# 1dayac/spades_for_blackbird

Hardware: AMD Instinct MI355X
Metric: distinct k-mers/sec (k=21, 150 bp synthetic reads, count only) (higher is better)
Workload: dtype u64

## Files before the change

spades_for_blackbird_amd/build.py:

```python
import os
import subprocess
import sys
from concurrent.futures import ThreadPoolExecutor

HERE = os.path.dirname(os.path.abspath(__file__))
CSRC = os.path.join(HERE, "csrc")
LIB = os.path.join(HERE, "libbbk.so")
SOURCES = ["pool.hip", "context.hip", "scan.hip", "sort.hip", "unique.hip", "msd.hip", "superk.hip", "reads.hip", "count.hip", "extindex.hip", "tipclip.hip", "atclip.hip", "readfilter.hip", "unitigs.hip", "unitigs_write.hip", "edgeprof.hip", "kmerprof.hip", "hamclust.hip", "kmerstat.hip", "subclust.hip", "expand.hip", "readcorrect.hip", "hreads.hip", "readprint.hip", "group.hip", "fastqparse.hip", "kmerfilter.hip"]
HEADERS = ["bbk_internal.h", "block_scan.h", "kmer_ops.h", "extwalk.h", "msd.h", "msd_part.h", "msd_bucket.h", "msd_narrow_a.h", "msd_stage_b.h", "msd_bucket_tail.h", "accum.h", "arena.h", "select.h", "unitigs.h", "hammer.h", "hammer_files.h", "readcorrect_host.hpp", os.path.join("..", "host", "hammer_reads.hpp"), "gfa_graph.h", os.path.join("..", "..", "include", "bbk.h")]
ARCH = "gfx950"
FLAGS = ["-O3", "-std=c++17", "-fPIC", "--offload-arch=" + ARCH, "-fopenmp", "-Wall", "-Wno-unused-function"]


def _hipcc():
    for c in (os.environ.get("HIPCC"), "/opt/rocm/bin/hipcc", "hipcc"):
        if c and (os.path.isabs(c) and os.path.exists(c) or not os.path.isabs(c)):
            return c
    raise RuntimeError("hipcc not found")


def _stale(target, deps):
    if not os.path.exists(target):
        return True
    t = os.path.getmtime(target)
# ... 119 lines not shown
```

spades_for_blackbird_amd/csrc/msd.hip:

```cpp
#include <hip/hip_runtime.h>

#include <algorithm>
#include <chrono>
#include <cmath>
#include <cstdio>
#include <cstdlib>
#include <cstring>
#include <optional>
#include <type_traits>
#include <utility>
#include <vector>

#include "bbk_internal.h"
#include "kmer_ops.h"
#include "msd.h"
#include "msd.h"

#include "msd_part.h"
#include "msd_bucket.h"
#include "msd_narrow_a.h"
#include "msd_stage_b.h"

namespace bbk {

// ... 518 lines not shown
                         v.slots.as<uint32_t>(), v.off.as<uint64_t>(), v.seg.as<uint16_t>(), vdesc.template as<uint2>(),
                         v.stride, v.hb, Mv, L1, cur1.as<uint32_t>(), bufA.as<Key<1>>());
            }
            if (v.n_extra) {
                TileMap Me = M1;
                Me.n = 2 * v.n_extra;
                const uint32_t nte = (uint32_t)((Me.n + kPartTileK - 1) / kPartTileK);
                R.template scatter_keys<true>(false, "k_part_l1", rec_bytes(v.n_extra) + rec_bytes(Me.n), nte,
                                              v.extra.as<Key<W>>(), nullptr, Me, L1, cur1.as<uint32_t>(),
                                              bufA.as<Key<W>>(), nullptr);
            }
        }

        void level1_late_tag(BucketView &v) {
            constexpr uint32_t kpt = (uint32_t)kLtThreads * kLt1Items / 2;
            const size_t lds = lt_smem(kLt1Items, (size_t)kViewSpan * (4 + 2));
            ctx->add_stat("stat_late_tag", (double)N);
            const auto [vdesc, nt] = view_tiles(v, kpt);
            if (nt)
                R.launch(k_part_view_lt<false>, "k_part_view", (double)v.D * 4 + 2.0 * (double)v.D * 4, nt, kLtThreads, lds,
                         v.slots.as<uint32_t>(), v.off.as<uint64_t>(), v.seg.as<uint16_t>(), vdesc.template as<uint2>(),
                         v.stride, v.hb, (const uint64_t *)nullptr, v.D, (int)R.expand_k, L1, cur1.as<uint32_t>(),
                         bufA.as<uint32_t>());
            if (v.n_extra) {
                const uint32_t nte = (uint32_t)((v.n_extra + kpt - 1) / kpt);
                R.launch(k_part_view_lt<true>, "k_part_l1", (double)v.n_extra * 8 + 2.0 * (double)v.n_extra * 4, nte,
                         kLtThreads, lds, (const uint32_t *)nullptr, (const uint64_t *)nullptr, (const uint16_t *)nullptr,
                         (const uint2 *)nullptr, 0u, 0, v.extra.as<uint64_t>(), v.n_extra, (int)R.expand_k, L1,
                         cur1.as<uint32_t>(), bufA.as<uint32_t>());
            }
        }
// ... 1042 lines not shown
```

spades_for_blackbird_amd/csrc/msd_narrow_a.h:

```cpp
#pragma once

namespace bbk {

constexpr int kNwBins1 = 1024;
__device__ inline uint32_t nw_mix(uint32_t lo) {
    uint32_t t = lo * 0x9E3779B1u;
    t ^= t >> 15;
    t *= 0x85EBCA6Bu;
    t ^= t >> 13;
    return t;
}
__device__ inline uint32_t nw_slot(uint32_t t) { return (t * 0x27D4EB2Fu) >> 19; }
__device__ inline uint32_t nw_bin1(uint32_t hi, uint32_t t, int hb) { return (t >> 22) ^ (hi << (10 - hb)); }
__device__ inline uint32_t nw_p2(uint32_t t) { return t << 10; }
__device__ inline uint32_t nw_bin2(uint32_t t, uint32_t nb) {
#ifdef BBK_AB_NW_BIN2_MULHI
    return __umulhi(nw_p2(t), nb);
#else
    return __umul24(t & 0x3FFFFFu, nb) >> 22;
#endif
}
__device__ inline uint64_t nw_key(uint32_t bin1, uint32_t lo, int hb) {
    const uint32_t hi = (bin1 ^ (nw_mix(lo) >> 22)) >> (10 - hb);
    return ((uint64_t)hi << 32) | lo;
// ... 127 lines not shown
        for (int i = 0; i < CH; ++i) lo[r * CH + i] = l8[i];
#pragma unroll
        for (int i = 0; i < 3; ++i) bins[r * 3 + i] = b3[i];
        masks[r * 2] = m2[0];
        masks[r * 2 + 1] = m2[1];
        cnts |= cnt << (4 * r);
    }
}

template <bool HAS_VAL>
__global__ __launch_bounds__(kNwThreads) __attribute__((amdgpu_waves_per_eu(BBK_NW_WAVES, BBK_NW_WAVES))) void k_part_reads_narrow(ReadSrc S, PartLevel L, uint32_t ntiles,
                                                                 const RdTile *__restrict__ tiles_arg,
                                                                 uint32_t *__restrict__ cursor,
                                                                 uint32_t *__restrict__ out, uint32_t *__restrict__ vout) {
    constexpr int NT = kNwThreads, CH = 8, MAXB = kNwBins1, ITEMS = CH * NwCfg<HAS_VAL>::ROUNDS;
    constexpr int MW = NwCfg<HAS_VAL>::TILE / 64;
    extern __shared__ __attribute__((aligned(16))) unsigned char smem[];
    uint32_t *lhist = reinterpret_cast<uint32_t *>(smem);
    uint2 *tab = reinterpret_cast<uint2 *>(smem);
    uint32_t *lstart = lhist + 2 * MAXB;
    uint32_t *scan_tmp = lstart + MAXB;
    unsigned long long *mark = reinterpret_cast<unsigned long long *>(scan_tmp + 64);
    uint16_t *mbase = reinterpret_cast<uint16_t *>(mark + MW);
    uint16_t *nz = mbase + MW;
    unsigned char *U = reinterpret_cast<unsigned char *>(nz + MAXB);
    int32_t *s_rel = reinterpret_cast<int32_t *>(U);
    int32_t *s_wrel = s_rel + (kRdSlots + 2);
    uint32_t *s_len = reinterpret_cast<uint32_t *>(s_wrel + (kRdSlots + 2));
    uint64_t *s_words = reinterpret_cast<uint64_t *>(s_len + (kRdSlots + 2));
    uint32_t *stage = reinterpret_cast<uint32_t *>(U);
    uint8_t *vstage = reinterpret_cast<uint8_t *>(stage + NwCfg<HAS_VAL>::TILE);

    uint32_t tid = threadIdx.x;
    const uint32_t k_ = (uint32_t)S.k;
    const int hb = L.narrow_hb;
    uint32_t xcc = 0;
    if (L.xcd_shift) {
        asm volatile("s_getreg_b32 %0, hwreg(HW_REG_XCC_ID)" : "=s"(xcc));
        xcc &= (1u << L.xcd_shift) - 1u;
    }
#ifdef BBK_PHASE_PROF
    unsigned long long t_prev = clock64();
#else
    const unsigned long long t_prev = 0;
    (void)t_prev;
#endif
// ... 16 lines not shown
    };

#ifdef BBK_NW_TILES_VIA_STRUCT
    const RdTile *tiles = S.tiles;
    (void)tiles_arg;
#else
    const RdTile *__restrict__ tiles = tiles_arg;
#endif
    uint32_t tile = blockIdx.x;
    if (tile >= ntiles) return;
    RdTile T = tiles[tile];
    Pre Q{0, 0, 0, 0, 0};
    prefetch(T, Q);
    for (;;) {
        asm volatile("" : "+v"(tid));
        const int lane = tid & 63, wave = tid >> 6;
        const uint32_t tile_next = tile + gridDim.x;
        const bool more = tile_next < ntiles;
        RdTile Tn = T;
        if (more) Tn = tiles[tile_next];

        const uint64_t c0 = (uint64_t)tile * NwCfg<HAS_VAL>::CHUNKS;
        const uint64_t left = S.n_chunks - c0;
        const uint32_t nch = left < (uint64_t)NwCfg<HAS_VAL>::CHUNKS ? (uint32_t)left : (uint32_t)NwCfg<HAS_VAL>::CHUNKS;
        const uint32_t r0 = T.r0, nr = T.nr;
        const uint64_t wbase = T.wbase;
        const bool fast = staged_ok(T);
        lhist[tid] = 0;
        if (tid < 2 * MW) reinterpret_cast<uint32_t *>(mark)[tid] = 0u;
        if (fast) {
            if (tid <= nr) s_rel[tid] = (int32_t)(int64_t)(Q.coff - c0);
            if (tid < nr) {
                s_wrel[tid] = (int32_t)(int64_t)(Q.woff - wbase);
                s_len[tid] = Q.len;
            }
            if (tid < T.wspan) s_words[tid] = Q.w0;
            if (tid + NT < T.wspan) s_words[tid + NT] = Q.w1;
        }
        __syncthreads();
        BBK_PH(5, 0, t_prev);

        uint32_t lo[ITEMS], bins[3 * NwCfg<HAS_VAL>::ROUNDS], masks[2 * NwCfg<HAS_VAL>::ROUNDS], cnts;
        if (fast) nw_extract<true, HAS_VAL>(S, L, k_, tid, nch, c0, r0, nr, s_rel, s_wrel, s_len, s_words, lhist, lo, bins, masks, cnts);
        else nw_extract<false, HAS_VAL>(S, L, k_, tid, nch, c0, r0, nr, s_rel, s_wrel, s_len, s_words, lhist, lo, bins, masks, cnts);
        __syncthreads();
        BBK_PH(5, 1, t_prev);

        const uint32_t c = lhist[tid];
        uint32_t incl = c;
        incl = wave_scan_incl(incl);
        const unsigned long long nzb = __ballot(c != 0);
        if (lane == 63) scan_tmp[wave] = incl | ((uint32_t)__popcll(nzb) << 16);
        __syncthreads();
        uint32_t before, total;
        wave_totals<NT / 64>(scan_tmp, lane, wave, before, total);
        const uint32_t staged = total & 0xFFFFu;
        const uint32_t ex = (before & 0xFFFFu) + incl - c;
        const uint32_t myr = (before >> 16) + (uint32_t)__popcll(nzb & ((1ull << lane) - 1ull));
        lstart[tid] = ex;
        uint32_t greserve = 0;
        if (c) {
            greserve = atomicAdd(&cursor[(tid << L.xcd_shift) + xcc], c);
            nz[myr] = (uint16_t)tid;
            atomicOr(&mark[ex >> 6], 1ull << (ex & 63u));
        }
        __syncthreads();
        BBK_PH(5, 2, t_prev);
#pragma unroll
        for (int i = 0; i < ITEMS; ++i) {
            const int r = i / CH, j = i % CH;
            if ((uint32_t)j < ((cnts >> (4 * r)) & 15u)) {
                const uint32_t bin = (bins[r * 3 + j / 3] >> (10 * (j % 3))) & 1023u;
                const uint32_t pos = atomicAdd(&lstart[bin], 1u);
                stage[pos] = lo[i];
                if (HAS_VAL) vstage[pos] = (uint8_t)(masks[r * 2 + (j >> 2)] >> (8 * (j & 3)));
            }
        }
        asm volatile("" : "+v"(greserve));
        if (c) {
            const uint64_t slot_end = L.xcd_shift ? (uint64_t)tid * L.slot_stride + (uint64_t)(xcc + 1u) * L.sub_cap
                                                  : (uint64_t)tid * L.slot_stride + L.slot_cap;
            const int64_t room = (int64_t)slot_end - (int64_t)greserve;
            tab[myr] = make_uint2(greserve - ex,
                                  (uint32_t)(int32_t)(room < -(int64_t)0x7FFF0000 ? -(int64_t)0x7FFF0000 : room) + ex);
        }
        if (wave == 0) {
            constexpr int WPL = (MW + 63) / 64;
            uint32_t pw[WPL], tot = 0;
#pragma unroll
            for (int j = 0; j < WPL; ++j) {
                const int idx = lane * WPL + j;
                pw[j] = tot;
                tot += idx < MW ? (uint32_t)__popcll(mark[idx]) : 0u;
            }
            uint32_t inc2 = tot;
            inc2 = wave_scan_incl(inc2);
            const uint32_t lb = inc2 - tot;
#pragma unroll
            for (int j = 0; j < WPL; ++j) {
                const int idx = lane * WPL + j;
                if (idx < MW) mbase[idx] = (uint16_t)(lb + pw[j]);
            }
        }
        __syncthreads();
        BBK_PH(5, 3, t_prev);
        if (more) prefetch(Tn, Q);
        else Q = Pre{0, 0, 0, 0, 0};
        const unsigned long long upto = (2ull << lane) - 1ull;
        const unsigned long long *wmark = mark + wave;
        const uint16_t *wmbase = mbase + wave;
        uint32_t full = 0;
#pragma unroll
        for (int i = 0; i < ITEMS; ++i) {
            const uint32_t pos = (uint32_t)i * NT + tid;
            if (pos < staged) {
                const uint32_t r = (uint32_t)wmbase[i * (NT / 64)] + (uint32_t)__popcll(wmark[i * (NT / 64)] & upto) - 1u;
                unsigned long long e = reinterpret_cast<const unsigned long long *>(tab)[r];
                const uint32_t rec = stage[pos];
                asm volatile("" : "+v"(e));
                if ((int32_t)pos >= (int32_t)(uint32_t)(e >> 32)) {
                    full |= 1u << i;
                } else {
                    const uint32_t g = (uint32_t)e + pos;
                    out[g] = rec;
                    if (HAS_VAL) vout[g] = vstage[pos];
                }
            }
        }
        if (full) {
#pragma unroll 1
            for (int i = 0; i < ITEMS; ++i) {
                if ((full >> i) & 1u) {
                    const uint32_t pos = (uint32_t)i * NT + tid;
                    const uint32_t r = (uint32_t)wmbase[i * (NT / 64)] + (uint32_t)__popcll(wmark[i * (NT / 64)] & upto) - 1u;
                    const uint32_t sp = atomicAdd(L.spill_count, 1u);
                    if (sp < L.spill_cap) {
                        reinterpret_cast<uint64_t *>(L.spill_keys)[sp] = nw_key(nz[r], stage[pos], hb);
                        if (HAS_VAL) L.spill_vals[sp] = vstage[pos];
                    }
                }
            }
        }
        BBK_PH(5, 4, t_prev);
#ifdef BBK_PHASE_PROF
        if (threadIdx.x == 0) atomicAdd(&g_phase[5][7], 1ull);
#endif
        if (!more) break;
        __syncthreads();
        tile = tile_next;
        T = Tn;
    }
}

static size_t part_reads_narrow_smem(bool has_val) {
    const size_t tables = sizeof(uint32_t) * 3 * (kRdSlots + 2) + sizeof(uint64_t) * (kRdWords + 1 + 2);
    const size_t tile = has_val ? NwCfg<true>::TILE : NwCfg<false>::TILE;
    const size_t stage = tile * (has_val ? 5 : 4);
    const size_t fixed = sizeof(uint32_t) * (3 * kNwBins1 + 64) + (tile / 64) * (8 + 2) + (size_t)kNwBins1 * 2;
    return fixed + std::max(tables, stage);
}

constexpr int kNw2Threads = 1024;
template <bool HAS_VAL>
struct Nw2Cfg {
    static constexpr int ITEMS = HAS_VAL ? 8 : 12;
    static constexpr int TILE = kNw2Threads * ITEMS;
};

template <bool HAS_VAL>
__global__ __launch_bounds__(kNw2Threads) void k_part_narrow2(const uint32_t *__restrict__ in, const uint32_t *__restrict__ vin,
                                                             const uint4 *__restrict__ desc, PartLevel L,
                                                             uint32_t *__restrict__ cursor, uint32_t *__restrict__ out,
                                                             uint32_t *__restrict__ vout) {
    constexpr int NT = kNw2Threads, ITEMS = Nw2Cfg<HAS_VAL>::ITEMS, MAXB = kMaxBins;
// ... 429 lines not shown
```

spades_for_blackbird_amd/csrc/msd_stage_b.h:

```cpp
#pragma once

#include "msd_bucket_tail.h"

namespace bbk {

__global__ void k_bucket_base(const uint32_t *__restrict__ seg_nb2, const uint32_t *__restrict__ seg_bin, uint32_t nseg,
                              uint32_t nbuckets, int b1, int w0bits, uint64_t *__restrict__ base) {
    const uint32_t g = blockIdx.x * blockDim.x + threadIdx.x;
    if (g >= nbuckets) return;
    const uint32_t lo = last_le(seg_bin, nseg, g);
    const uint64_t P = 1ull << (32 - b1), nb = seg_nb2[lo], j = g - seg_bin[lo];
    const uint64_t p = lo * P + (j * P + nb - 1) / nb;
    base[g] = w0bits > 32 ? p << (w0bits - 32) : 0ull;
}

template <int NT, int ITEMS>
__global__ __launch_bounds__(NT) __attribute__((amdgpu_waves_per_eu(8, 8))) void k_bucket_dist_nb(const uint32_t *__restrict__ buf, const uint64_t *__restrict__ base,
                                                       BucketArgs A) {
    constexpr int CAP = NT * ITEMS;
    constexpr int NWAVES = NT / 64;
    constexpr int DB = DistBins<1, 0>::N;
    constexpr int BPT = DB / NT;
    extern __shared__ __attribute__((aligned(16))) unsigned char smem[];
    uint32_t *bins = reinterpret_cast<uint32_t *>(smem);
// ... 328 lines not shown
            keep = !kmer_less_nucl<1>(kmer_rc<1>(x, k), x);
        }
        const uint64_t bal = __ballot(keep);
        uint32_t base = 0;
        if (lane == 0 && bal) base = atomicAdd(count, (uint32_t)__popcll(bal));
        base = __shfl(base, 0);
        const uint64_t at = (uint64_t)base + __popcll(bal & ((1ull << lane) - 1ull));
        if (keep && at < cap) out[at] = x.w[0];
    }
}

constexpr int kLtThreads = 1024;
constexpr int kLt1Items = 14;
constexpr int kLt2Items = 12;

struct LtLds {
    uint32_t *lhist;
    uint2 *tab;
    uint32_t *lstart, *scan_tmp;
    unsigned long long *mark;
    uint16_t *mbase, *nz;
    uint32_t *stage;
};
template <int ITEMS>
__device__ __forceinline__ LtLds lt_lds(unsigned char *smem) {
    constexpr int MW = kLtThreads * ITEMS / 64;
    LtLds S;
    S.lhist = reinterpret_cast<uint32_t *>(smem);
    S.tab = reinterpret_cast<uint2 *>(smem);
    S.lstart = S.lhist + 2 * kMaxBins;
    S.scan_tmp = S.lstart + kMaxBins;
    S.mark = reinterpret_cast<unsigned long long *>(S.scan_tmp + 64);
    S.mbase = reinterpret_cast<uint16_t *>(S.mark + MW);
    S.nz = S.mbase + MW;
    S.stage = reinterpret_cast<uint32_t *>(S.nz + kMaxBins);
    return S;
}
static size_t lt_smem(int items, size_t more) {
    const size_t tile = (size_t)kLtThreads * items;
    return sizeof(uint32_t) * (3 * kMaxBins + 64) + (tile / 64) * (8 + 2) + (size_t)kMaxBins * 2 + tile * 4 + more;
}

__device__ inline uint64_t lt_tagged(uint32_t seg, uint32_t lo, int lobits, int k) {
    Key<1> x;
    x.w[0] = ((uint64_t)seg << lobits) | lo;
    return x.w[0] | (__umul64hi(xxh3_64<1>(x), 16ull) << (2 * k));
}

template <int ITEMS, class KeyOf>
__device__ __forceinline__ void lt_tail(const LtLds &S, const uint32_t (&lo)[ITEMS], const uint32_t (&bins)[ITEMS / 2],
                                        uint32_t nb, uint32_t *__restrict__ cur, uint64_t slot_end, uint32_t rec_or,
                                        const PartLevel &L, uint32_t *__restrict__ out, KeyOf key_of) {
    constexpr int NT = kLtThreads, MW = NT * ITEMS / 64;
    static_assert(ITEMS % 2 == 0 && ITEMS <= 32 && NT * ITEMS < 65536, "packed bins, one bit per item, 16-bit positions");
    const uint32_t tid = threadIdx.x;
    const int lane = tid & 63, wave = tid >> 6;
    const uint32_t c = tid < nb ? S.lhist[tid] : 0u;
    uint32_t incl = c;
    incl = wave_scan_incl(incl);
    const unsigned long long nzb = __ballot(c != 0);
    if (lane == 63) S.scan_tmp[wave] = incl | ((uint32_t)__popcll(nzb) << 16);
    __syncthreads();
    uint32_t before, total;
    wave_totals<NT / 64>(S.scan_tmp, lane, wave, before, total);
    const uint32_t staged = total & 0xFFFFu;
    const uint32_t ex = (before & 0xFFFFu) + incl - c;
    const uint32_t myr = (before >> 16) + (uint32_t)__popcll(nzb & ((1ull << lane) - 1ull));
    S.lstart[tid] = ex;
    uint32_t greserve = 0;
    if (c) {
        greserve = atomicAdd(cur, c);
        S.nz[myr] = (uint16_t)tid;
        atomicOr(&S.mark[ex >> 6], 1ull << (ex & 63u));
    }
    __syncthreads();
#pragma unroll
    for (int i = 0; i < ITEMS; ++i) {
        const uint32_t bin = (bins[i >> 1] >> (16 * (i & 1))) & 0xFFFFu;
        if (bin != 0xFFFFu) {
            const uint32_t pos = atomicAdd(&S.lstart[bin], 1u);
            S.stage[pos] = lo[i];
        }
    }
    asm volatile("" : "+v"(greserve));
    if (c) {
        const int64_t room = (int64_t)slot_end - (int64_t)greserve;
        S.tab[myr] = make_uint2(greserve - ex, (uint32_t)(int32_t)(room < -(int64_t)0x7FFF0000 ? -(int64_t)0x7FFF0000 : room) + ex);
    }
    if (wave == 0) {
        constexpr int WPL = (MW + 63) / 64;
        uint32_t pw[WPL], tot = 0;
#pragma unroll
        for (int j = 0; j < WPL; ++j) {
            const int idx = lane * WPL + j;
            pw[j] = tot;
            tot += idx < MW ? (uint32_t)__popcll(S.mark[idx]) : 0u;
        }
        uint32_t inc2 = tot;
        inc2 = wave_scan_incl(inc2);
        const uint32_t lb = inc2 - tot;
#pragma unroll
        for (int j = 0; j < WPL; ++j) {
            const int idx = lane * WPL + j;
            if (idx < MW) S.mbase[idx] = (uint16_t)(lb + pw[j]);
        }
    }
    __syncthreads();
    const unsigned long long upto = (2ull << lane) - 1ull;
    const unsigned long long *wmark = S.mark + wave;
    const uint16_t *wmbase = S.mbase + wave;
    uint32_t full = 0;
#pragma unroll
    for (int i = 0; i < ITEMS; ++i) {
        const uint32_t pos = (uint32_t)i * NT + tid;
        if (pos < staged) {
            const uint32_t r = (uint32_t)wmbase[i * (NT / 64)] + (uint32_t)__popcll(wmark[i * (NT / 64)] & upto) - 1u;
            unsigned long long e = reinterpret_cast<const unsigned long long *>(S.tab)[r];
            const uint32_t rec = S.stage[pos];
            asm volatile("" : "+v"(e));
            if ((int32_t)pos >= (int32_t)(uint32_t)(e >> 32)) full |= 1u << i;
            else out[(uint32_t)e + pos] = rec | rec_or;
        }
    }
    if (full) {
#pragma unroll 1
        for (int i = 0; i < ITEMS; ++i) {
            if ((full >> i) & 1u) {
                const uint32_t pos = (uint32_t)i * NT + tid;
                const uint32_t r = (uint32_t)wmbase[i * (NT / 64)] + (uint32_t)__popcll(wmark[i * (NT / 64)] & upto) - 1u;
                const uint32_t sp = atomicAdd(L.spill_count, 1u);
                if (sp < L.spill_cap) reinterpret_cast<uint64_t *>(L.spill_keys)[sp] = key_of((uint32_t)S.nz[r], S.stage[pos]);
            }
        }
    }
}

template <bool DENSE>
__global__ __launch_bounds__(kLtThreads) __attribute__((amdgpu_waves_per_eu(8, 8))) void k_part_view_lt(
    const uint32_t *__restrict__ slots, const uint64_t *__restrict__ off, const uint16_t *__restrict__ seg,
    const uint2 *__restrict__ vdesc, uint32_t stride, int hb, const uint64_t *__restrict__ dense, uint64_t nkeys_all, int k,
    PartLevel L, uint32_t *__restrict__ cursor, uint32_t *__restrict__ out) {
    constexpr int NT = kLtThreads, ITEMS = kLt1Items, KPT = NT * ITEMS / 2, MW = NT * ITEMS / 64;
    extern __shared__ __attribute__((aligned(16))) unsigned char smem[];
    const LtLds S = lt_lds<ITEMS>(smem);
    uint32_t *toff = S.stage + NT * ITEMS;
    uint16_t *tseg = reinterpret_cast<uint16_t *>(toff + kViewSpan);
    const uint32_t tid = threadIdx.x;
    uint32_t xcc = 0;
    if (L.xcd_shift) {
        asm volatile("s_getreg_b32 %0, hwreg(HW_REG_XCC_ID)" : "=s"(xcc));
        xcc &= (1u << L.xcd_shift) - 1u;
    }
    const int lobits = 2 * k - 10;
    const uint32_t lomask = lobits >= 32 ? 0xFFFFFFFFu : (1u << lobits) - 1u;
    const uint64_t c0 = (uint64_t)blockIdx.x * KPT;
    const uint64_t left = nkeys_all - c0;
    const uint32_t nkeys = left < (uint64_t)KPT ? (uint32_t)left : (uint32_t)KPT;
    uint32_t b0 = 0, span = 0;
    bool staged_tab = false;
    if (!DENSE) {
        const uint2 d = vdesc[blockIdx.x];
        b0 = d.x;
        span = d.y - d.x + 1u;
        staged_tab = span <= (uint32_t)kViewSpan;
        if (staged_tab && tid < span) {
            toff[tid] = (uint32_t)off[b0 + tid];
            tseg[tid] = seg[b0 + tid];
        }
    }
    S.lhist[tid] = 0;
    if (tid < 2 * MW) reinterpret_cast<uint32_t *>(S.mark)[tid] = 0u;
    __syncthreads();

    uint64_t x[ITEMS / 2];
    if (DENSE) {
#pragma unroll
        for (int j = 0; j < ITEMS / 2; ++j) {
            const uint32_t cl = (uint32_t)(j * NT) + tid;
            x[j] = dense[c0 + (cl < nkeys ? cl : nkeys - 1u)];
        }
    } else {
        uint32_t w[ITEMS / 2], sg[ITEMS / 2];
#pragma unroll
        for (int j = 0; j < ITEMS / 2; ++j) {
            const uint32_t cl = (uint32_t)(j * NT) + tid;
            const uint32_t c = (uint32_t)c0 + (cl < nkeys ? cl : nkeys - 1u);
            uint32_t b, base;
            if (staged_tab) {
                uint32_t i = 0, hi = span;
                while (hi - i > 1) {
                    const uint32_t mid = (i + hi) >> 1;
                    if (toff[mid] <= c) i = mid;
                    else hi = mid;
                }
                b = b0 + i;
                base = toff[i];
                sg[j] = tseg[i];
            } else {
                b = view_bucket(off, b0, b0 + span, c);
                base = (uint32_t)off[b];
                sg[j] = seg[b];
            }
            w[j] = slots[(size_t)b * stride + (c - base)];
        }
#pragma unroll
        for (int j = 0; j < ITEMS / 2; ++j) x[j] = nw_key(sg[j], w[j], hb);
    }
    uint32_t lo[ITEMS], bins[ITEMS / 2];
#pragma unroll
    for (int j = 0; j < ITEMS / 2; ++j) {
        Key<1> a;
        a.w[0] = x[j];
        const uint64_t r = kmer_rc<1>(a, k).w[0];
        const uint32_t ba = (uint32_t)(x[j] >> lobits), br = (uint32_t)(r >> lobits);
        lo[2 * j] = (uint32_t)x[j] & lomask;
        lo[2 * j + 1] = (uint32_t)r & lomask;
        bins[j] = 0xFFFFFFFFu;
        if ((uint32_t)(j * NT) + tid < nkeys) {
            bins[j] = ba | (br << 16);
            atomicAdd(&S.lhist[ba], 1u);
            atomicAdd(&S.lhist[br], 1u);
        }
    }
    __syncthreads();
    const uint64_t slot_end = (uint64_t)tid * L.slot_stride + (L.xcd_shift ? (uint64_t)(xcc + 1u) * L.sub_cap : (uint64_t)L.slot_cap);
    lt_tail<ITEMS>(S, lo, bins, (uint32_t)kMaxBins, &cursor[(tid << L.xcd_shift) + xcc], slot_end, 0u, L, out,
                   [&](uint32_t bin, uint32_t rec) { return lt_tagged(bin, rec, lobits, k); });
}

__global__ __launch_bounds__(kLtThreads) __attribute__((amdgpu_waves_per_eu(8, 8))) void k_part_lt2(
    const uint32_t *__restrict__ in, const uint4 *__restrict__ desc, int k, PartLevel L, uint32_t *__restrict__ cursor,
    uint32_t *__restrict__ out) {
    constexpr int NT = kLtThreads, ITEMS = kLt2Items, MW = NT * ITEMS / 64;
    extern __shared__ __attribute__((aligned(16))) unsigned char smem[];
    const LtLds S = lt_lds<ITEMS>(smem);
    const uint32_t tid = threadIdx.x;
    const uint4 d = desc[blockIdx.x];
    const uint32_t begin = d.x, count = d.y, nb = d.z & 0xFFFFu, sgm = d.z >> 16, gbin0 = d.w;
    if (count == 0) return;
    const int lobits = 2 * k - 10;
    const uint32_t nsub = nb >> 4;
    const uint64_t segbits = (uint64_t)sgm << lobits;
    S.lhist[tid] = 0;
    if (tid < 2 * MW) reinterpret_cast<uint32_t *>(S.mark)[tid] = 0u;
    __syncthreads();
    uint32_t lo[ITEMS], bins[ITEMS / 2];
#pragma unroll
    for (int i = 0; i < ITEMS; ++i) {
        const uint32_t local = (uint32_t)i * NT + tid;
        lo[i] = in[begin + (local < count ? local : count - 1u)];
    }
#pragma unroll
    for (int i = 0; i < ITEMS; ++i) asm volatile("" : "+v"(lo[i]));
#pragma unroll
    for (int i = 0; i < ITEMS; ++i) {
        Key<1> x;
        x.w[0] = segbits | lo[i];
        const uint32_t tag = (uint32_t)__umul64hi(xxh3_64<1>(x), 16ull);
        const uint32_t b = tag * nsub + __umulhi(lo[i] << (32 - lobits), nsub);
        const bool valid = (uint32_t)i * NT + tid < count;
        if (valid) atomicAdd(&S.lhist[b], 1u);
        const uint32_t b16 = valid ? b : 0xFFFFu;
        if (i & 1) bins[i >> 1] |= b16 << 16;
        else bins[i >> 1] = b16;
    }
    __syncthreads();
    const uint64_t slot_end = (uint64_t)(gbin0 + tid) * L.slot_stride + L.slot_cap;
    lt_tail<ITEMS>(S, lo, bins, nb, &cursor[gbin0 + tid], slot_end, (uint32_t)segbits, L, out,
                   [&](uint32_t, uint32_t rec) { return lt_tagged(sgm, rec, lobits, k); });
}

__global__ void k_bucket_base_lt(const uint32_t *__restrict__ seg_nb2, const uint32_t *__restrict__ seg_bin, uint32_t nseg,
                                 uint32_t nbuckets, int lobits, int k, uint64_t *__restrict__ base,
                                 uint32_t *__restrict__ perm) {
    const uint32_t g = blockIdx.x * blockDim.x + threadIdx.x;
    if (g >= nbuckets) return;
    const uint32_t lo = last_le(seg_bin, nseg, g);
    const uint32_t nsub = seg_nb2[lo] >> 4, r = g - seg_bin[lo], tag = r / nsub, j = r - tag * nsub;
    const uint64_t q = (((uint64_t)j << lobits) + nsub - 1u) / nsub;
    base[g] = ((uint64_t)tag << (2 * k)) | ((uint64_t)lo << lobits) | q;
    perm[g] = tag * (nbuckets >> 4) + (seg_bin[lo] >> 4) + j;
}

__global__ void k_lt_fill_perm(const uint32_t *__restrict__ cursor, const uint32_t *__restrict__ perm, uint32_t n,
// ... 55 lines not shown
```

Baseline: 31.39 billion.

## Share a mark-rank scatter tail across partition kernels using mbcnt ranks

Moves the duplicated histogram/scan/scatter tail of the narrow and late-tag partition kernels into one shared mark_tail helper. The helper stores per-word mark bits with a precomputed prefix and finds ranks via mbcnt, and adds a fast path that writes straight through 64-bit address tables when no bucket overflows. The late-tag view lookup also replaces its per-key binary search over the staged offset table with a rank query on a bitmap of run starts. These aim to cut LDS reads, divergent search loops and per-store checks, at the cost of a larger LDS layout, some extra setup work and more complex code.

```diff
diff --git a/spades_for_blackbird_amd/build.py b/spades_for_blackbird_amd/build.py
--- a/spades_for_blackbird_amd/build.py
+++ b/spades_for_blackbird_amd/build.py
@@ -7,7 +7,7 @@
 CSRC = os.path.join(HERE, "csrc")
 LIB = os.path.join(HERE, "libbbk.so")
 SOURCES = ["pool.hip", "context.hip", "scan.hip", "sort.hip", "unique.hip", "msd.hip", "superk.hip", "reads.hip", "count.hip", "extindex.hip", "tipclip.hip", "atclip.hip", "readfilter.hip", "unitigs.hip", "unitigs_write.hip", "edgeprof.hip", "kmerprof.hip", "hamclust.hip", "kmerstat.hip", "subclust.hip", "expand.hip", "readcorrect.hip", "hreads.hip", "readprint.hip", "group.hip", "fastqparse.hip", "kmerfilter.hip"]
-HEADERS = ["bbk_internal.h", "block_scan.h", "kmer_ops.h", "extwalk.h", "msd.h", "msd_part.h", "msd_bucket.h", "msd_narrow_a.h", "msd_stage_b.h", "msd_bucket_tail.h", "accum.h", "arena.h", "select.h", "unitigs.h", "hammer.h", "hammer_files.h", "readcorrect_host.hpp", os.path.join("..", "host", "hammer_reads.hpp"), "gfa_graph.h", os.path.join("..", "..", "include", "bbk.h")]
+HEADERS = ["bbk_internal.h", "block_scan.h", "kmer_ops.h", "extwalk.h", "msd.h", "msd_part.h", "msd_bucket.h", "msd_narrow_a.h", "msd_stage_b.h", "msd_bucket_tail.h", "msd_mark_tail.h", "accum.h", "arena.h", "select.h", "unitigs.h", "hammer.h", "hammer_files.h", "readcorrect_host.hpp", os.path.join("..", "host", "hammer_reads.hpp"), "gfa_graph.h", os.path.join("..", "..", "include", "bbk.h")]
 ARCH = "gfx950"
 FLAGS = ["-O3", "-std=c++17", "-fPIC", "--offload-arch=" + ARCH, "-fopenmp", "-Wall", "-Wno-unused-function"]
 
diff --git a/spades_for_blackbird_amd/csrc/msd.hip b/spades_for_blackbird_amd/csrc/msd.hip
--- a/spades_for_blackbird_amd/csrc/msd.hip
+++ b/spades_for_blackbird_amd/csrc/msd.hip
@@ -556,7 +556,7 @@
 
         void level1_late_tag(BucketView &v) {
             constexpr uint32_t kpt = (uint32_t)kLtThreads * kLt1Items / 2;
-            const size_t lds = lt_smem(kLt1Items, (size_t)kViewSpan * (4 + 2));
+            const size_t lds = lt_smem(kLt1Items, lt_view_tables());
             ctx->add_stat("stat_late_tag", (double)N);
             const auto [vdesc, nt] = view_tiles(v, kpt);
             if (nt)
diff --git a/spades_for_blackbird_amd/csrc/msd_mark_tail.h b/spades_for_blackbird_amd/csrc/msd_mark_tail.h
--- /dev/null
+++ b/spades_for_blackbird_amd/csrc/msd_mark_tail.h
@@ -0,0 +1,217 @@
+#pragma once
+
+#include <cstdint>
+
+#if defined(__HIPCC__) || defined(__CUDACC__)
+#define BBK_MARK_HD __host__ __device__
+#else
+#define BBK_MARK_HD
+#endif
+
+namespace bbk {
+
+struct alignas(16) MarkWord {
+    uint32_t lo, hi;
+    uint32_t before;
+    uint32_t pad;
+};
+
+BBK_MARK_HD inline uint32_t mark_words(uint32_t positions) { return (positions + 63u) >> 6; }
+BBK_MARK_HD inline uint32_t mark_slot32(uint32_t start) {
+    const uint32_t s = start - 1u;
+    return ((s >> 6) << 2) | ((s >> 5) & 1u);
+}
+BBK_MARK_HD inline uint32_t mark_bit32(uint32_t start) { return 1u << ((start - 1u) & 31u); }
+BBK_MARK_HD inline uint32_t mark_count(uint32_t lo, uint32_t hi) {
+    return (uint32_t)__builtin_popcount(lo) + (uint32_t)__builtin_popcount(hi);
+}
+BBK_MARK_HD inline uint32_t mark_rank(uint32_t lo, uint32_t hi, uint32_t before, uint32_t lane) {
+#if defined(__HIP_DEVICE_COMPILE__)
+    (void)lane;
+    return __builtin_amdgcn_mbcnt_hi(hi, __builtin_amdgcn_mbcnt_lo(lo, before));
+#else
+    const uint32_t mlo = lane >= 32u ? 0xFFFFFFFFu : (1u << lane) - 1u;
+    const uint32_t mhi = lane <= 32u ? 0u : (1u << (lane - 32u)) - 1u;
+    return before + mark_count(lo & mlo, hi & mhi);
+#endif
+}
+
+BBK_MARK_HD inline uint32_t view_run_start(uint64_t off_i, uint64_t c0) { return off_i > c0 ? (uint32_t)(off_i - c0) : 0u; }
+BBK_MARK_HD inline bool view_bucket_live(uint32_t i, uint32_t span, uint64_t off_i, uint64_t off_next) {
+    return i + 1u == span || off_next != off_i;
+}
+
+#if defined(__HIPCC__)
+
+typedef __attribute__((address_space(1))) uint32_t MarkGlobalWord;
+
+struct MarkLds {
+    uint32_t *lhist;
+    unsigned long long *tab;
+    uint32_t *lstart, *scan_tmp;
+    MarkWord *mw;
+    uint16_t *nz;
+    uint32_t *stage;
+    uint8_t *vstage;
+};
+template <int TILE>
+__device__ __forceinline__ MarkLds mark_lds(unsigned char *smem) {
+    MarkLds S;
+    S.lhist = reinterpret_cast<uint32_t *>(smem);
+    S.tab = reinterpret_cast<unsigned long long *>(smem);
+    S.lstart = S.lhist + 2 * kMaxBins;
+    S.scan_tmp = S.lstart + kMaxBins;
+    S.mw = reinterpret_cast<MarkWord *>(S.scan_tmp + 64);
+    S.nz = reinterpret_cast<uint16_t *>(S.mw + TILE / 64);
+    S.stage = reinterpret_cast<uint32_t *>(S.nz + kMaxBins);
+    S.vstage = reinterpret_cast<uint8_t *>(S.stage + TILE);
+    return S;
+}
+static size_t mark_smem(size_t tile) {
+    return sizeof(uint32_t) * (3 * kMaxBins + 64) + (tile / 64) * sizeof(MarkWord) + (size_t)kMaxBins * 2;
+}
+template <int TILE>
+__device__ __forceinline__ void mark_clear(const MarkLds &S, uint32_t tid) {
+    static_assert(4 * (TILE / 64) <= kMaxBins, "one 32-bit word of the marks per thread");
+    S.lhist[tid] = 0;
+    if (tid < 4u * (TILE / 64)) reinterpret_cast<uint32_t *>(S.mw)[tid] = 0u;
+}
+
+template <int MW>
+__device__ __forceinline__ void mark_prefix(MarkWord *mw, int lane) {
+    constexpr int WPL = (MW + 63) / 64;
+    uint32_t pw[WPL], tot = 0;
+#pragma unroll
+    for (int j = 0; j < WPL; ++j) {
+        const int idx = lane * WPL + j;
+        pw[j] = tot;
+        if (idx < MW) {
+            const uint2 m = *reinterpret_cast<const uint2 *>(&mw[idx]);
+            tot += mark_count(m.x, m.y);
+        }
+    }
+    uint32_t inc2 = tot;
+    inc2 = wave_scan_incl(inc2);
+    const uint32_t lb = inc2 - tot;
+#pragma unroll
+    for (int j = 0; j < WPL; ++j) {
+        const int idx = lane * WPL + j;
+        if (idx < MW) mw[idx].before = lb + pw[j];
+    }
+}
+
+template <int NT>
+__device__ __forceinline__ uint32_t mark_rank_at(const MarkWord *wmw, int i, int lane) {
+    const uint4 m = *reinterpret_cast<const uint4 *>(&wmw[i * (NT / 64)]);
+    return mark_rank(m.x, m.y, m.z, (uint32_t)lane);
+}
+
+template <int TILE, int ITEMS, bool HAS_VAL, class BinOf, class ValOf, class KeyOf, class Hook>
+__device__ __forceinline__ void mark_tail(const MarkLds &S, const uint32_t (&lo)[ITEMS], uint32_t tid, uint32_t nb,
+                                          uint32_t *__restrict__ cur, uint64_t slot_end, uint32_t rec_or, const PartLevel &L,
+                                          uint32_t *__restrict__ out, uint32_t *__restrict__ vout, BinOf bin_of_item,
+                                          ValOf val_of, KeyOf key_of, Hook before_stores) {
+    constexpr int NT = kMaxBins, MW = TILE / 64;
+    static_assert(ITEMS <= 32 && TILE <= NT * ITEMS && NT * ITEMS < 65536, "one bit per item, 16-bit positions");
+    const int lane = tid & 63, wave = tid >> 6;
+    const uint32_t c = tid < nb ? S.lhist[tid] : 0u;
+    uint32_t incl = c;
+    incl = wave_scan_incl(incl);
+    const unsigned long long nzb = __ballot(c != 0);
+    if (lane == 63) S.scan_tmp[wave] = incl | ((uint32_t)__popcll(nzb) << 16);
+    if (tid == 0) S.scan_tmp[32] = 0;
+    __syncthreads();
+    uint32_t before, total;
+    wave_totals<NT / 64>(S.scan_tmp, lane, wave, before, total);
+    const uint32_t staged = total & 0xFFFFu;
+    const uint32_t ex = (before & 0xFFFFu) + incl - c;
+    const uint32_t myr = (before >> 16) + (uint32_t)__popcll(nzb & ((1ull << lane) - 1ull));
+    S.lstart[tid] = ex;
+    uint32_t greserve = 0;
+    if (c) {
+        greserve = atomicAdd(cur, c);
+        S.nz[myr] = (uint16_t)tid;
+        if (ex) atomicOr(&reinterpret_cast<uint32_t *>(S.mw)[mark_slot32(ex)], mark_bit32(ex));
+    }
+    __syncthreads();
+#pragma unroll
+    for (int i = 0; i < ITEMS; ++i) {
+        const uint32_t bin = bin_of_item(i);
+        if (bin != 0xFFFFFFFFu) {
+            const uint32_t pos = atomicAdd(&S.lstart[bin], 1u);
+            S.stage[pos] = lo[i];
+            if (HAS_VAL) S.vstage[pos] = (uint8_t)val_of(i);
+        }
+    }
+    asm volatile("" : "+v"(greserve));
+    int64_t room = 0;
+    if (c) {
+        room = (int64_t)slot_end - (int64_t)greserve;
+        S.tab[myr] = (unsigned long long)(uintptr_t)out + 4ull * (unsigned long long)((int64_t)greserve - (int64_t)ex);
+        if (room < (int64_t)c) S.scan_tmp[32] = 1;
+    }
+    if (wave == 0) mark_prefix<MW>(S.mw, lane);
+    __syncthreads();
+    before_stores();
+    const MarkWord *wmw = S.mw + wave;
+#ifdef BBK_AB_NO_MARK_FAST
+    const bool over = true;
+#else
+    const bool over = __builtin_amdgcn_readfirstlane((int)S.scan_tmp[32]) != 0;
+#endif
+    if (!over) {
+        const unsigned long long vdelta = (unsigned long long)((uintptr_t)vout - (uintptr_t)out);
+#pragma unroll
+        for (int i = 0; i < ITEMS; ++i) {
+            const uint32_t pos = (uint32_t)i * NT + tid;
+            if (pos < staged) {
+                const uint32_t r = mark_rank_at<NT>(wmw, i, lane);
+                const unsigned long long a = S.tab[r] + ((unsigned long long)pos << 2);
+                *reinterpret_cast<MarkGlobalWord *>(a) = S.stage[pos] | rec_or;
+                if (HAS_VAL) *reinterpret_cast<MarkGlobalWord *>(a + vdelta) = S.vstage[pos];
+            }
+        }
+        return;
+    }
+    if (c) {
+        S.tab[myr] = (unsigned long long)(greserve - ex) |
+                     ((unsigned long long)((uint32_t)(int32_t)(room < -(int64_t)0x7FFF0000 ? -(int64_t)0x7FFF0000 : room) + ex) << 32);
+    }
+    __syncthreads();
+    uint32_t full = 0;
+#pragma unroll
+    for (int i = 0; i < ITEMS; ++i) {
+        const uint32_t pos = (uint32_t)i * NT + tid;
+        if (pos < staged) {
+            const uint32_t r = mark_rank_at<NT>(wmw, i, lane);
+            unsigned long long e = S.tab[r];
+            const uint32_t rec = S.stage[pos];
+            asm volatile("" : "+v"(e));
+            if ((int32_t)pos >= (int32_t)(uint32_t)(e >> 32)) {
+                full |= 1u << i;
+            } else {
+                const uint32_t g = (uint32_t)e + pos;
+                out[g] = rec | rec_or;
+                if (HAS_VAL) vout[g] = S.vstage[pos];
+            }
+        }
+    }
+    if (full) {
+#pragma unroll 1
+        for (int i = 0; i < ITEMS; ++i) {
+            if ((full >> i) & 1u) {
+                const uint32_t pos = (uint32_t)i * NT + tid;
+                const uint32_t r = mark_rank_at<NT>(wmw, i, lane);
+                const uint32_t sp = atomicAdd(L.spill_count, 1u);
+                if (sp < L.spill_cap) {
+                    reinterpret_cast<uint64_t *>(L.spill_keys)[sp] = key_of((uint32_t)S.nz[r], S.stage[pos]);
+                    if (HAS_VAL) L.spill_vals[sp] = S.vstage[pos];
+                }
+            }
+        }
+    }
+}
+
+#endif
+
+}
diff --git a/spades_for_blackbird_amd/csrc/msd_narrow_a.h b/spades_for_blackbird_amd/csrc/msd_narrow_a.h
--- a/spades_for_blackbird_amd/csrc/msd_narrow_a.h
+++ b/spades_for_blackbird_amd/csrc/msd_narrow_a.h
@@ -1,4 +1,6 @@
 #pragma once
+
+#include "msd_mark_tail.h"
 
 namespace bbk {
 
@@ -165,22 +167,14 @@
                                                                  uint32_t *__restrict__ cursor,
                                                                  uint32_t *__restrict__ out, uint32_t *__restrict__ vout) {
     constexpr int NT = kNwThreads, CH = 8, MAXB = kNwBins1, ITEMS = CH * NwCfg<HAS_VAL>::ROUNDS;
-    constexpr int MW = NwCfg<HAS_VAL>::TILE / 64;
     extern __shared__ __attribute__((aligned(16))) unsigned char smem[];
-    uint32_t *lhist = reinterpret_cast<uint32_t *>(smem);
-    uint2 *tab = reinterpret_cast<uint2 *>(smem);
-    uint32_t *lstart = lhist + 2 * MAXB;
-    uint32_t *scan_tmp = lstart + MAXB;
-    unsigned long long *mark = reinterpret_cast<unsigned long long *>(scan_tmp + 64);
-    uint16_t *mbase = reinterpret_cast<uint16_t *>(mark + MW);
-    uint16_t *nz = mbase + MW;
-    unsigned char *U = reinterpret_cast<unsigned char *>(nz + MAXB);
+    const MarkLds ML = mark_lds<NwCfg<HAS_VAL>::TILE>(smem);
+    uint32_t *lhist = ML.lhist;
+    unsigned char *U = reinterpret_cast<unsigned char *>(ML.stage);
     int32_t *s_rel = reinterpret_cast<int32_t *>(U);
     int32_t *s_wrel = s_rel + (kRdSlots + 2);
     uint32_t *s_len = reinterpret_cast<uint32_t *>(s_wrel + (kRdSlots + 2));
     uint64_t *s_words = reinterpret_cast<uint64_t *>(s_len + (kRdSlots + 2));
-    uint32_t *stage = reinterpret_cast<uint32_t *>(U);
-    uint8_t *vstage = reinterpret_cast<uint8_t *>(stage + NwCfg<HAS_VAL>::TILE);
 
     uint32_t tid = threadIdx.x;
     const uint32_t k_ = (uint32_t)S.k;
@@ -227,7 +221,6 @@
     prefetch(T, Q);
     for (;;) {
         asm volatile("" : "+v"(tid));
-        const int lane = tid & 63, wave = tid >> 6;
         const uint32_t tile_next = tile + gridDim.x;
         const bool more = tile_next < ntiles;
         RdTile Tn = T;
@@ -239,8 +232,7 @@
         const uint32_t r0 = T.r0, nr = T.nr;
         const uint64_t wbase = T.wbase;
         const bool fast = staged_ok(T);
-        lhist[tid] = 0;
-        if (tid < 2 * MW) reinterpret_cast<uint32_t *>(mark)[tid] = 0u;
+        mark_clear<NwCfg<HAS_VAL>::TILE>(ML, tid);
         if (fast) {
             if (tid <= nr) s_rel[tid] = (int32_t)(int64_t)(Q.coff - c0);
             if (tid < nr) {
@@ -259,101 +251,21 @@
         __syncthreads();
         BBK_PH(5, 1, t_prev);
 
-        const uint32_t c = lhist[tid];
-        uint32_t incl = c;
-        incl = wave_scan_incl(incl);
-        const unsigned long long nzb = __ballot(c != 0);
-        if (lane == 63) scan_tmp[wave] = incl | ((uint32_t)__popcll(nzb) << 16);
-        __syncthreads();
-        uint32_t before, total;
-        wave_totals<NT / 64>(scan_tmp, lane, wave, before, total);
-        const uint32_t staged = total & 0xFFFFu;
-        const uint32_t ex = (before & 0xFFFFu) + incl - c;
-        const uint32_t myr = (before >> 16) + (uint32_t)__popcll(nzb & ((1ull << lane) - 1ull));
-        lstart[tid] = ex;
-        uint32_t greserve = 0;
-        if (c) {
-            greserve = atomicAdd(&cursor[(tid << L.xcd_shift) + xcc], c);
-            nz[myr] = (uint16_t)tid;
-            atomicOr(&mark[ex >> 6], 1ull << (ex & 63u));
-        }
-        __syncthreads();
-        BBK_PH(5, 2, t_prev);
-#pragma unroll
-        for (int i = 0; i < ITEMS; ++i) {
-            const int r = i / CH, j = i % CH;
-            if ((uint32_t)j < ((cnts >> (4 * r)) & 15u)) {
-                const uint32_t bin = (bins[r * 3 + j / 3] >> (10 * (j % 3))) & 1023u;
-                const uint32_t pos = atomicAdd(&lstart[bin], 1u);
-                stage[pos] = lo[i];
-                if (HAS_VAL) vstage[pos] = (uint8_t)(masks[r * 2 + (j >> 2)] >> (8 * (j & 3)));
-            }
-        }
-        asm volatile("" : "+v"(greserve));
-        if (c) {
-            const uint64_t slot_end = L.xcd_shift ? (uint64_t)tid * L.slot_stride + (uint64_t)(xcc + 1u) * L.sub_cap
-                                                  : (uint64_t)tid * L.slot_stride + L.slot_cap;
-            const int64_t room = (int64_t)slot_end - (int64_t)greserve;
-            tab[myr] = make_uint2(greserve - ex,
-                                  (uint32_t)(int32_t)(room < -(int64_t)0x7FFF0000 ? -(int64_t)0x7FFF0000 : room) + ex);
-        }
-        if (wave == 0) {
-            constexpr int WPL = (MW + 63) / 64;
-            uint32_t pw[WPL], tot = 0;
-#pragma unroll
-            for (int j = 0; j < WPL; ++j) {
-                const int idx = lane * WPL + j;
-                pw[j] = tot;
-                tot += idx < MW ? (uint32_t)__popcll(mark[idx]) : 0u;
-            }
-            uint32_t inc2 = tot;
-            inc2 = wave_scan_incl(inc2);
-            const uint32_t lb = inc2 - tot;
-#pragma unroll
-            for (int j = 0; j < WPL; ++j) {
-                const int idx = lane * WPL + j;
-                if (idx < MW) mbase[idx] = (uint16_t)(lb + pw[j]);
-            }
-        }
-        __syncthreads();
-        BBK_PH(5, 3, t_prev);
-        if (more) prefetch(Tn, Q);
-        else Q = Pre{0, 0, 0, 0, 0};
-        const unsigned long long upto = (2ull << lane) - 1ull;
-        const unsigned long long *wmark = mark + wave;
-        const uint16_t *wmbase = mbase + wave;
-        uint32_t full = 0;
-#pragma unroll
-        for (int i = 0; i < ITEMS; ++i) {
-            const uint32_t pos = (uint32_t)i * NT + tid;
-            if (pos < staged) {
-                const uint32_t r = (uint32_t)wmbase[i * (NT / 64)] + (uint32_t)__popcll(wmark[i * (NT / 64)] & upto) - 1u;
-                unsigned long long e = reinterpret_cast<const unsigned long long *>(tab)[r];
-                const uint32_t rec = stage[pos];
-                asm volatile("" : "+v"(e));
-                if ((int32_t)pos >= (int32_t)(uint32_t)(e >> 32)) {
-                    full |= 1u << i;
-                } else {
-                    const uint32_t g = (uint32_t)e + pos;
-                    out[g] = rec;
-                    if (HAS_VAL) vout[g] = vstage[pos];
-                }
-            }
-        }
-        if (full) {
-#pragma unroll 1
-            for (int i = 0; i < ITEMS; ++i) {
-                if ((full >> i) & 1u) {
-                    const uint32_t pos = (uint32_t)i * NT + tid;
-                    const uint32_t r = (uint32_t)wmbase[i * (NT / 64)] + (uint32_t)__popcll(wmark[i * (NT / 64)] & upto) - 1u;
-                    const uint32_t sp = atomicAdd(L.spill_count, 1u);
-                    if (sp < L.spill_cap) {
-                        reinterpret_cast<uint64_t *>(L.spill_keys)[sp] = nw_key(nz[r], stage[pos], hb);
-                        if (HAS_VAL) L.spill_vals[sp] = vstage[pos];
-                    }
-                }
-            }
-        }
+        const uint64_t slot_end = L.xcd_shift ? (uint64_t)tid * L.slot_stride + (uint64_t)(xcc + 1u) * L.sub_cap
+                                              : (uint64_t)tid * L.slot_stride + L.slot_cap;
+        mark_tail<NwCfg<HAS_VAL>::TILE, ITEMS, HAS_VAL>(
+            ML, lo, tid, (uint32_t)MAXB, &cursor[(tid << L.xcd_shift) + xcc], slot_end, 0u, L, out, vout,
+            [&](int i) {
+                const int r = i / CH, j = i % CH;
+                return (uint32_t)j < ((cnts >> (4 * r)) & 15u) ? (bins[r * 3 + j / 3] >> (10 * (j % 3))) & 1023u : 0xFFFFFFFFu;
+            },
+            [&](int i) { return masks[(i / CH) * 2 + ((i % CH) >> 2)] >> (8 * (i & 3)); },
+            [&](uint32_t bin, uint32_t rec) { return nw_key(bin, rec, hb); },
+            [&]() {
+                BBK_PH(5, 3, t_prev);
+                if (more) prefetch(Tn, Q);
+                else Q = Pre{0, 0, 0, 0, 0};
+            });
         BBK_PH(5, 4, t_prev);
 #ifdef BBK_PHASE_PROF
         if (threadIdx.x == 0) atomicAdd(&g_phase[5][7], 1ull);
@@ -369,8 +281,7 @@
     const size_t tables = sizeof(uint32_t) * 3 * (kRdSlots + 2) + sizeof(uint64_t) * (kRdWords + 1 + 2);
     const size_t tile = has_val ? NwCfg<true>::TILE : NwCfg<false>::TILE;
     const size_t stage = tile * (has_val ? 5 : 4);
-    const size_t fixed = sizeof(uint32_t) * (3 * kNwBins1 + 64) + (tile / 64) * (8 + 2) + (size_t)kNwBins1 * 2;
-    return fixed + std::max(tables, stage);
+    return mark_smem(tile) + std::max(tables, stage);
 }
 
 constexpr int kNw2Threads = 1024;
diff --git a/spades_for_blackbird_amd/csrc/msd_stage_b.h b/spades_for_blackbird_amd/csrc/msd_stage_b.h
--- a/spades_for_blackbird_amd/csrc/msd_stage_b.h
+++ b/spades_for_blackbird_amd/csrc/msd_stage_b.h
@@ -366,31 +366,12 @@
 constexpr int kLt1Items = 14;
 constexpr int kLt2Items = 12;
 
-struct LtLds {
-    uint32_t *lhist;
-    uint2 *tab;
-    uint32_t *lstart, *scan_tmp;
-    unsigned long long *mark;
-    uint16_t *mbase, *nz;
-    uint32_t *stage;
-};
-template <int ITEMS>
-__device__ __forceinline__ LtLds lt_lds(unsigned char *smem) {
-    constexpr int MW = kLtThreads * ITEMS / 64;
-    LtLds S;
-    S.lhist = reinterpret_cast<uint32_t *>(smem);
-    S.tab = reinterpret_cast<uint2 *>(smem);
-    S.lstart = S.lhist + 2 * kMaxBins;
-    S.scan_tmp = S.lstart + kMaxBins;
-    S.mark = reinterpret_cast<unsigned long long *>(S.scan_tmp + 64);
-    S.mbase = reinterpret_cast<uint16_t *>(S.mark + MW);
-    S.nz = S.mbase + MW;
-    S.stage = reinterpret_cast<uint32_t *>(S.nz + kMaxBins);
-    return S;
-}
 static size_t lt_smem(int items, size_t more) {
     const size_t tile = (size_t)kLtThreads * items;
-    return sizeof(uint32_t) * (3 * kMaxBins + 64) + (tile / 64) * (8 + 2) + (size_t)kMaxBins * 2 + tile * 4 + more;
+    return mark_smem(tile) + tile * 4 + more;
+}
+static size_t lt_view_tables() {
+    return ((size_t)kLtThreads * kLt1Items / 2 / 64) * sizeof(MarkWord) + (size_t)kViewSpan * sizeof(uint2);
 }
 
 __device__ inline uint64_t lt_tagged(uint32_t seg, uint32_t lo, int lobits, int k) {
@@ -399,92 +380,10 @@
     return x.w[0] | (__umul64hi(xxh3_64<1>(x), 16ull) << (2 * k));
 }
 
-template <int ITEMS, class KeyOf>
-__device__ __forceinline__ void lt_tail(const LtLds &S, const uint32_t (&lo)[ITEMS], const uint32_t (&bins)[ITEMS / 2],
-                                        uint32_t nb, uint32_t *__restrict__ cur, uint64_t slot_end, uint32_t rec_or,
-                                        const PartLevel &L, uint32_t *__restrict__ out, KeyOf key_of) {
-    constexpr int NT = kLtThreads, MW = NT * ITEMS / 64;
-    static_assert(ITEMS % 2 == 0 && ITEMS <= 32 && NT * ITEMS < 65536, "packed bins, one bit per item, 16-bit positions");
-    const uint32_t tid = threadIdx.x;
-    const int lane = tid & 63, wave = tid >> 6;
-    const uint32_t c = tid < nb ? S.lhist[tid] : 0u;
-    uint32_t incl = c;
-    incl = wave_scan_incl(incl);
-    const unsigned long long nzb = __ballot(c != 0);
-    if (lane == 63) S.scan_tmp[wave] = incl | ((uint32_t)__popcll(nzb) << 16);
-    __syncthreads();
-    uint32_t before, total;
-    wave_totals<NT / 64>(S.scan_tmp, lane, wave, before, total);
-    const uint32_t staged = total & 0xFFFFu;
-    const uint32_t ex = (before & 0xFFFFu) + incl - c;
-    const uint32_t myr = (before >> 16) + (uint32_t)__popcll(nzb & ((1ull << lane) - 1ull));
-    S.lstart[tid] = ex;
-    uint32_t greserve = 0;
-    if (c) {
-        greserve = atomicAdd(cur, c);
-        S.nz[myr] = (uint16_t)tid;
-        atomicOr(&S.mark[ex >> 6], 1ull << (ex & 63u));
-    }
-    __syncthreads();
-#pragma unroll
-    for (int i = 0; i < ITEMS; ++i) {
-        const uint32_t bin = (bins[i >> 1] >> (16 * (i & 1))) & 0xFFFFu;
-        if (bin != 0xFFFFu) {
-            const uint32_t pos = atomicAdd(&S.lstart[bin], 1u);
-            S.stage[pos] = lo[i];
-        }
-    }
-    asm volatile("" : "+v"(greserve));
-    if (c) {
-        const int64_t room = (int64_t)slot_end - (int64_t)greserve;
-        S.tab[myr] = make_uint2(greserve - ex, (uint32_t)(int32_t)(room < -(int64_t)0x7FFF0000 ? -(int64_t)0x7FFF0000 : room) + ex);
-    }
-    if (wave == 0) {
-        constexpr int WPL = (MW + 63) / 64;
-        uint32_t pw[WPL], tot = 0;
-#pragma unroll
-        for (int j = 0; j < WPL; ++j) {
-            const int idx = lane * WPL + j;
-            pw[j] = tot;
-            tot += idx < MW ? (uint32_t)__popcll(S.mark[idx]) : 0u;
-        }
-        uint32_t inc2 = tot;
-        inc2 = wave_scan_incl(inc2);
-        const uint32_t lb = inc2 - tot;
-#pragma unroll
-        for (int j = 0; j < WPL; ++j) {
-            const int idx = lane * WPL + j;
-            if (idx < MW) S.mbase[idx] = (uint16_t)(lb + pw[j]);
-        }
-    }
-    __syncthreads();
-    const unsigned long long upto = (2ull << lane) - 1ull;
-    const unsigned long long *wmark = S.mark + wave;
-    const uint16_t *wmbase = S.mbase + wave;
-    uint32_t full = 0;
-#pragma unroll
-    for (int i = 0; i < ITEMS; ++i) {
-        const uint32_t pos = (uint32_t)i * NT + tid;
-        if (pos < staged) {
-            const uint32_t r = (uint32_t)wmbase[i * (NT / 64)] + (uint32_t)__popcll(wmark[i * (NT / 64)] & upto) - 1u;
-            unsigned long long e = reinterpret_cast<const unsigned long long *>(S.tab)[r];
-            const uint32_t rec = S.stage[pos];
-            asm volatile("" : "+v"(e));
-            if ((int32_t)pos >= (int32_t)(uint32_t)(e >> 32)) full |= 1u << i;
-            else out[(uint32_t)e + pos] = rec | rec_or;
-        }
-    }
-    if (full) {
-#pragma unroll 1
-        for (int i = 0; i < ITEMS; ++i) {
-            if ((full >> i) & 1u) {
-                const uint32_t pos = (uint32_t)i * NT + tid;
-                const uint32_t r = (uint32_t)wmbase[i * (NT / 64)] + (uint32_t)__popcll(wmark[i * (NT / 64)] & upto) - 1u;
-                const uint32_t sp = atomicAdd(L.spill_count, 1u);
-                if (sp < L.spill_cap) reinterpret_cast<uint64_t *>(L.spill_keys)[sp] = key_of((uint32_t)S.nz[r], S.stage[pos]);
-            }
-        }
-    }
+template <int ITEMS>
+__device__ __forceinline__ uint32_t lt_bin(const uint32_t (&bins)[ITEMS / 2], int i) {
+    const uint32_t bin = (bins[i >> 1] >> (16 * (i & 1))) & 0xFFFFu;
+    return bin != 0xFFFFu ? bin : 0xFFFFFFFFu;
 }
 
 template <bool DENSE>
@@ -492,11 +391,12 @@
     const uint32_t *__restrict__ slots, const uint64_t *__restrict__ off, const uint16_t *__restrict__ seg,
     const uint2 *__restrict__ vdesc, uint32_t stride, int hb, const uint64_t *__restrict__ dense, uint64_t nkeys_all, int k,
     PartLevel L, uint32_t *__restrict__ cursor, uint32_t *__restrict__ out) {
-    constexpr int NT = kLtThreads, ITEMS = kLt1Items, KPT = NT * ITEMS / 2, MW = NT * ITEMS / 64;
+    constexpr int NT = kLtThreads, ITEMS = kLt1Items, KPT = NT * ITEMS / 2, VW = KPT / 64;
+    static_assert(KPT % 64 == 0 && VW <= 128, "whole words of marks, two per lane of one wave");
     extern __shared__ __attribute__((aligned(16))) unsigned char smem[];
-    const LtLds S = lt_lds<ITEMS>(smem);
-    uint32_t *toff = S.stage + NT * ITEMS;
-    uint16_t *tseg = reinterpret_cast<uint16_t *>(toff + kViewSpan);
+    const MarkLds S = mark_lds<NT * ITEMS>(smem);
+    MarkWord *vmw = reinterpret_cast<MarkWord *>(S.stage + NT * ITEMS);
+    uint2 *vent = reinterpret_cast<uint2 *>(vmw + VW);
     const uint32_t tid = threadIdx.x;
     uint32_t xcc = 0;
     if (L.xcd_shift) {
@@ -515,13 +415,37 @@
         b0 = d.x;
         span = d.y - d.x + 1u;
         staged_tab = span <= (uint32_t)kViewSpan;
-        if (staged_tab && tid < span) {
-            toff[tid] = (uint32_t)off[b0 + tid];
-            tseg[tid] = seg[b0 + tid];
-        }
-    }
-    S.lhist[tid] = 0;
-    if (tid < 2 * MW) reinterpret_cast<uint32_t *>(S.mark)[tid] = 0u;
+        if (staged_tab && tid < 64u) {
+            uint64_t o = 0, on = 0;
+            uint32_t sg = 0;
+            if (tid < span) {
+                o = off[b0 + tid];
+                if (tid + 1u < span) on = off[b0 + tid + 1u];
+                sg = seg[b0 + tid];
+            }
+#ifdef BBK_AB_VIEW_SEARCH
+            (void)on;
+            if (tid < span) vent[tid] = make_uint2((uint32_t)o, tid | (sg << 16));
+#else
+#pragma unroll
+            for (int j = 0; j < 2; ++j) {
+                const uint32_t idx = tid * 2u + (uint32_t)j;
+                if (idx < (uint32_t)VW) *reinterpret_cast<uint4 *>(&vmw[idx]) = make_uint4(0u, 0u, 0u, 0u);
+            }
+            __threadfence_block();
+            const bool live = tid < span && view_bucket_live(tid, span, o, on);
+            const unsigned long long lv = __ballot(live);
+            if (live) {
+                vent[__popcll(lv & ((1ull << tid) - 1ull))] = make_uint2((uint32_t)o, tid | (sg << 16));
+                const uint32_t start = view_run_start(o, c0);
+                if (start) atomicOr(&reinterpret_cast<uint32_t *>(vmw)[mark_slot32(start)], mark_bit32(start));
+            }
+            __threadfence_block();
+            mark_prefix<VW>(vmw, (int)tid);
+#endif
+        }
+    }
+    mark_clear<NT * ITEMS>(S, tid);
     __syncthreads();
 
     uint64_t x[ITEMS / 2];
@@ -539,15 +463,21 @@
             const uint32_t c = (uint32_t)c0 + (cl < nkeys ? cl : nkeys - 1u);
             uint32_t b, base;
             if (staged_tab) {
+#ifdef BBK_AB_VIEW_SEARCH
                 uint32_t i = 0, hi = span;
                 while (hi - i > 1) {
                     const uint32_t mid = (i + hi) >> 1;
-                    if (toff[mid] <= c) i = mid;
+                    if (vent[mid].x <= c) i = mid;
                     else hi = mid;
                 }
-                b = b0 + i;
-                base = toff[i];
-                sg[j] = tseg[i];
+                const uint2 e = vent[i];
+#else
+                const uint4 m = *reinterpret_cast<const uint4 *>(&vmw[j * (NT / 64) + (int)(tid >> 6)]);
+                const uint2 e = vent[mark_rank(m.x, m.y, m.z, tid & 63u)];
+#endif
+                b = b0 + (e.y & 0xFFFFu);
+                base = e.x;
+                sg[j] = e.y >> 16;
             } else {
                 b = view_bucket(off, b0, b0 + span, c);
                 base = (uint32_t)off[b];
@@ -576,16 +506,18 @@
     }
     __syncthreads();
     const uint64_t slot_end = (uint64_t)tid * L.slot_stride + (L.xcd_shift ? (uint64_t)(xcc + 1u) * L.sub_cap : (uint64_t)L.slot_cap);
-    lt_tail<ITEMS>(S, lo, bins, (uint32_t)kMaxBins, &cursor[(tid << L.xcd_shift) + xcc], slot_end, 0u, L, out,
-                   [&](uint32_t bin, uint32_t rec) { return lt_tagged(bin, rec, lobits, k); });
+    mark_tail<NT * ITEMS, ITEMS, false>(
+        S, lo, tid, (uint32_t)kMaxBins, &cursor[(tid << L.xcd_shift) + xcc], slot_end, 0u, L, out, nullptr,
+        [&](int i) { return lt_bin<ITEMS>(bins, i); }, [](int) { return 0u; },
+        [&](uint32_t bin, uint32_t rec) { return lt_tagged(bin, rec, lobits, k); }, []() {});
 }
 
 __global__ __launch_bounds__(kLtThreads) __attribute__((amdgpu_waves_per_eu(8, 8))) void k_part_lt2(
     const uint32_t *__restrict__ in, const uint4 *__restrict__ desc, int k, PartLevel L, uint32_t *__restrict__ cursor,
     uint32_t *__restrict__ out) {
-    constexpr int NT = kLtThreads, ITEMS = kLt2Items, MW = NT * ITEMS / 64;
+    constexpr int NT = kLtThreads, ITEMS = kLt2Items;
     extern __shared__ __attribute__((aligned(16))) unsigned char smem[];
-    const LtLds S = lt_lds<ITEMS>(smem);
+    const MarkLds S = mark_lds<NT * ITEMS>(smem);
     const uint32_t tid = threadIdx.x;
     const uint4 d = desc[blockIdx.x];
     const uint32_t begin = d.x, count = d.y, nb = d.z & 0xFFFFu, sgm = d.z >> 16, gbin0 = d.w;
@@ -593,8 +525,7 @@
     const int lobits = 2 * k - 10;
     const uint32_t nsub = nb >> 4;
     const uint64_t segbits = (uint64_t)sgm << lobits;
-    S.lhist[tid] = 0;
-    if (tid < 2 * MW) reinterpret_cast<uint32_t *>(S.mark)[tid] = 0u;
+    mark_clear<NT * ITEMS>(S, tid);
     __syncthreads();
     uint32_t lo[ITEMS], bins[ITEMS / 2];
 #pragma unroll
@@ -618,8 +549,10 @@
     }
     __syncthreads();
     const uint64_t slot_end = (uint64_t)(gbin0 + tid) * L.slot_stride + L.slot_cap;
-    lt_tail<ITEMS>(S, lo, bins, nb, &cursor[gbin0 + tid], slot_end, (uint32_t)segbits, L, out,
-                   [&](uint32_t, uint32_t rec) { return lt_tagged(sgm, rec, lobits, k); });
+    mark_tail<NT * ITEMS, ITEMS, false>(
+        S, lo, tid, nb, &cursor[gbin0 + tid], slot_end, (uint32_t)segbits, L, out, nullptr,
+        [&](int i) { return lt_bin<ITEMS>(bins, i); }, [](int) { return 0u; },
+        [&](uint32_t, uint32_t rec) { return lt_tagged(sgm, rec, lobits, k); }, []() {});
 }
 
 __global__ void k_bucket_base_lt(const uint32_t *__restrict__ seg_nb2, const uint32_t *__restrict__ seg_bin, uint32_t nseg,
```

Result: faster. 31.77 billion (median of 6 runs) (+1.2%).
